# the3cloud/zktls

Hardware: AMD Instinct MI355X
Metric: trace-cells/s (higher is better)
Workload: dtype u32

## Files before the change

### zktls_amd/csrc/context.cpp

```cpp
#include "context.h"
#include "poseidon2.cuh"

#include <atomic>
#include <mutex>
#include <vector>

#include <cstdio>
#include <cstdlib>
#include <cstring>
#include <string>

namespace zk {

extern std::atomic<int> g_live_contexts;

static thread_local std::string g_last_error;

void set_error(const std::string& msg) { g_last_error = msg; }
void fiber_tls_swap_error(std::string& err) { g_last_error.swap(err); }
int fail(int code, const std::string& msg) { g_last_error = msg; return code; }
int hip_fail(hipError_t e, const char* what) {
    g_last_error = std::string("HIP error ") + hipGetErrorName(e) + " (" + hipGetErrorString(e) + ") in " + what;
    (void)hipGetLastError();
    return e == hipErrorOutOfMemory ? ZKHIP_ERR_NOMEM : ZKHIP_ERR_HIP;
// ... 389 lines not shown
        }
        const BigPlan* fp;
        ZK_TRY(get_big_plan(ctx, log_n, 2, st, &fp));
        CombineArgs f = cm[0] ? combine_args(cm[t], width, dst, out_ld, width, log_n, fp) : combine_args(dst, out_ld, dst, out_ld, width, log_n, fp);
        if (cm[0]) { f.in_group_mul = 1; f.in_elem_mul = Np; } else { f.in_group_mul = R; f.in_elem_mul = 1; }
        f.out_group_mul = R; f.out_elem_mul = 1; f.bitrev_out = 1;
        ZK_HIP(launch_ntt_combine(f, ctx->stream));
    }
    return ZKHIP_OK;
}

constexpr int SMALL_LDE_MIN_LOG = 11, SMALL_LDE_MAX_LOG = 15, SMALL_LDE_DEFAULT_MAX_LOG = 13;
constexpr uint32_t SMALL_LDE_MIN_WIDTH = 128;
static int get_small_plan(zkhip_ctx* ctx, int log_n, const SmallPlan** out) {
    for (const SmallPlan& p : ctx->small_plans) if (p.log_n == log_n) { *out = &p; return ZKHIP_OK; }
    SmallPlan p;
    p.log_n = log_n;
    const size_t m = (size_t)1 << (log_n - 5);
    const uint32_t w = two_adic_generator(log_n);
    ZK_HIP(hipMalloc((void**)&p.tw_inv, m * 4));
    if (hipMalloc((void**)&p.tw_fwd, m * 4) != hipSuccess) { (void)hipFree(p.tw_inv); return fail(ZKHIP_ERR_HIP, "hipMalloc (small LDE tables)"); }
    hipError_t e = launch_pow_table(p.tw_inv, m, finv(w), MONTY_R1, ctx->stream);
    if (e == hipSuccess) e = launch_pow_table(p.tw_fwd, m, w, MONTY_R1, ctx->stream);
    if (e != hipSuccess) { (void)hipFree(p.tw_inv); (void)hipFree(p.tw_fwd); return hip_fail(e, "small LDE tables"); }
    ctx->small_plans.push_back(p);
    *out = &ctx->small_plans.back();
    return ZKHIP_OK;
}
static int get_small_pre(zkhip_ctx* ctx, int log_n, uint32_t shift, const uint32_t** out) {
    for (const SmallPre& p : ctx->small_pres) if (p.log_n == log_n && p.shift == shift) { *out = p.pre; return ZKHIP_OK; }
    SmallPre p;
    p.log_n = log_n; p.shift = shift;
    const size_t n = (size_t)1 << log_n;
    ZK_HIP(hipMalloc((void**)&p.pre, n * 4));
    const hipError_t e = launch_pow_table(p.pre, n, shift, finv(to_monty((uint32_t)n)), ctx->stream);
    if (e != hipSuccess) { (void)hipFree(p.pre); return hip_fail(e, "small LDE coset powers"); }
    ctx->small_pres.push_back(p);
    *out = p.pre;
    return ZKHIP_OK;
}
static int lde_small(zkhip_ctx* ctx, const uint32_t* in, size_t in_ld, uint32_t* out, size_t out_ld, int log_n, uint32_t width, int log_blowup,
                     uint32_t shift, bool* done) {
    *done = false;
    if (log_n < SMALL_LDE_MIN_LOG || log_n > SMALL_LDE_MAX_LOG || !ctx->lde_fusion) return ZKHIP_OK;
    int max_log = SMALL_LDE_DEFAULT_MAX_LOG;
    uint32_t min_width = SMALL_LDE_MIN_WIDTH;
#ifdef ZKHIP_AB_HOOKS
    if (const char* e = getenv("ZKHIP_LDE_SMALL")) { max_log = atoi(e); min_width = 1; }
#endif
    if (log_n > max_log || width < min_width) return ZKHIP_OK;
    const size_t n = (size_t)1 << log_n;
    const int B = 1 << log_blowup;
    LdeSmallArgs a{};
    a.in = in; a.in_ld = in_ld; a.out_ld = out_ld; a.ncols = width; a.cosets = (uint32_t)B;
    if (!lde_small_supported(a, log_n)) return ZKHIP_OK;
    const SmallPlan* sp;
    ZK_TRY(get_small_plan(ctx, log_n, &sp));
    a.tw_inv = sp->tw_inv; a.tw_fwd = sp->tw_fwd;
    const uint32_t wnb = two_adic_generator(log_n + log_blowup);
    for (int t = 0; t < B; t++) {
        ZK_TRY(get_small_pre(ctx, log_n, fmul(shift, fpow(wnb, (uint64_t)t)), &a.pre[t]));
        a.out[t] = out + (size_t)reverse_bits((uint32_t)t, log_blowup) * n * out_ld;
    }
    ZK_HIP(launch_lde_small(a, log_n, ctx->stream));
    *done = true;
    return ZKHIP_OK;
}

int op_coset_lde(zkhip_ctx* ctx, const uint32_t* in, size_t in_ld, uint32_t* out, size_t out_ld,
                 int log_n, uint32_t width, int log_blowup, uint32_t shift) {
    if (log_n < 0 || log_n > MAX_LOG_ROWS) return fail(ZKHIP_ERR_INVALID, "coset_lde: log_n must be in [0, 22]");
    if (log_n > BIG_INNER_LOG) {
        if (log_blowup < 0 || log_blowup > 4 || log_n + log_blowup > TWO_ADICITY) return fail(ZKHIP_ERR_INVALID, "coset_lde: bad log_blowup");
        if (width == 0 || in_ld < width || out_ld < width) return fail(ZKHIP_ERR_INVALID, "coset_lde: bad width / ld");
        return coset_lde_big(ctx, in, in_ld, out, out_ld, log_n, width, log_blowup, shift);
    }
    if (log_blowup < 0 || log_blowup > 4 || log_n + log_blowup > TWO_ADICITY) return fail(ZKHIP_ERR_INVALID, "coset_lde: bad log_blowup");
    if (width == 0 || in_ld < width || out_ld < width) return fail(ZKHIP_ERR_INVALID, "coset_lde: bad width / ld");
    if (log_n < 5) {
        void* coef_s;
        ZK_TRY(ctx_reserve(ctx, S_COEF, ((size_t)1 << log_n) * width * 4, &coef_s));
        ZK_HIP(launch_small_eval(in, in_ld, (uint32_t*)coef_s, width, log_n, log_n, width, finv(two_adic_generator(log_n)), MONTY_R1,
                                 finv(to_monty(1u << log_n)), 0, ctx->stream));
        ZK_HIP(launch_small_eval((const uint32_t*)coef_s, width, out, out_ld, log_n, log_n + log_blowup, width,
                                 two_adic_generator(log_n + log_blowup), shift, MONTY_R1, 1, ctx->stream));
        return ZKHIP_OK;
    }
    {
        bool done = false;
        ZK_TRY(lde_small(ctx, in, in_ld, out, out_ld, log_n, width, log_blowup, shift, &done));
        if (done) return ZKHIP_OK;
    }
    if (width > 32 && width % 32 != 0) {
        const uint32_t w32 = width & ~31u;
        ZK_TRY(op_coset_lde(ctx, in, in_ld, out, out_ld, log_n, w32, log_blowup, shift));
        return op_coset_lde(ctx, in + w32, in_ld, out + w32, out_ld, log_n, width - w32, log_blowup, shift);
    }
    const size_t n = (size_t)1 << log_n;
    const int B = 1 << log_blowup;
    int m1, m2;
    split(log_n, &m1, &m2);
    void* coef_v;
    ZK_TRY(ctx_reserve(ctx, S_COEF, n * width * 4, &coef_v));
    uint32_t* coef = (uint32_t*)coef_v;
    const uint32_t wnb = two_adic_generator(log_n + log_blowup);
    if (m1 == 0) {
        ZK_TRY(run_inverse(ctx, in, in_ld, coef, width, log_n, width, false));
        for (int t = 0; t < B; t++) {
            const uint32_t st = fmul(shift, fpow(wnb, (uint64_t)t));
            uint32_t* dst = out + (size_t)reverse_bits((uint32_t)t, log_blowup) * n * out_ld;
            const NttPlan* p;
            ZK_TRY(get_plan(ctx, log_n, 1, st, &p));
            NttPassArgs a = base_args(ctx, coef, width, dst, out_ld, width, false);
            a.num_tiles = 1; a.log_m = log_n; a.in_tile_mul = 0; a.in_stride = 1; a.out_tile_mul = 0; a.out_stride = 1;
            a.pre = p->pre; a.bitrev_out = 1;
            ZK_HIP(launch_ntt_pass(a, false, ctx->stream));
        }
        return ZKHIP_OK;
    }
    uint32_t* dsts[16];
    uint32_t shifts[16];
    for (int t = 0; t < B; t++) {
        shifts[t] = fmul(shift, fpow(wnb, (uint64_t)t));
        dsts[t] = out + (size_t)reverse_bits((uint32_t)t, log_blowup) * n * out_ld;
    }
    return lde_two_pass(ctx, in, in_ld, coef, width, dsts, out_ld, log_n, width, shifts, B);
}

int op_merkle_commit(zkhip_ctx* ctx, const MatDesc* mats, int nmats, int log_h, uint32_t* tree) {
    if (nmats < 1 || nmats > MAX_LEAF_MATS) return fail(ZKHIP_ERR_INVALID, "merkle_commit: 1..8 matrices");
    if (log_h < 0 || log_h > 30) return fail(ZKHIP_ERR_INVALID, "merkle_commit: bad log_h");
    LeafArgs la{};
    for (int m = 0; m < nmats; m++) la.mats[m] = mats[m];
    la.nmats = nmats; la.height = (uint64_t)1 << log_h; la.digests = tree;
    uint32_t* level = tree;
    uint64_t count = la.height;
    if (count > COOP_TOP_NODES && count <= coop_max_nodes()) {
        const uint32_t rest = count >= 4096 ? 128u : 32u;
        ZK_HIP(launch_hash_sub(la, (uint32_t)count / rest, ctx->stream));
        for (uint64_t c = count; c > rest; c >>= 1) level += 8 * c;
        ZK_HIP(launch_compress_top(level, rest, ctx->stream));
        return ZKHIP_OK;
    }
    ZK_HIP(launch_hash_rows(la, ctx->stream));
    while (count > COOP_TOP_NODES) {
        if (count <= coop_max_nodes()) {
            const uint32_t rest = count >= 4096 ? 128u : 32u;
            const uint32_t sub = (uint32_t)count / rest;
            ZK_HIP(launch_compress_sub(level, (uint32_t)count, sub, ctx->stream));
            for (uint64_t c = count; c > rest; c >>= 1) level += 8 * c;
            count = rest;
            break;
        }
        uint32_t* next = level + 8 * count;
        ZK_HIP(launch_compress_level(level, next, count / 2, ctx->stream));
        level = next; count >>= 1;
    }
    ZK_HIP(launch_compress_top(level, (uint32_t)count, ctx->stream));
    return ZKHIP_OK;
}

int op_merkle_commit_mixed(zkhip_ctx* ctx, const MatDesc* mats, const int* log_heights, int nmats, uint32_t* tree) {
    if (nmats < 1 || nmats > 32) return fail(ZKHIP_ERR_INVALID, "merkle_commit_mixed: 1..32 matrices");
    int log_h = 0;
    for (int m = 0; m < nmats; m++) {
        if (log_heights[m] < 0 || log_heights[m] > 30) return fail(ZKHIP_ERR_INVALID, "merkle_commit_mixed: bad height");
        if (log_heights[m] > log_h) log_h = log_heights[m];
    }
    auto gather = [&](int lh, LeafArgs& la) {
        la = LeafArgs{};
        for (int m = 0; m < nmats; m++)
            if (log_heights[m] == lh) {
                if (la.nmats == MAX_LEAF_MATS) return false;
                la.mats[la.nmats++] = mats[m];
            }
        la.height = (uint64_t)1 << lh;
        return true;
    };
    LeafArgs la;
    if (!gather(log_h, la)) return fail(ZKHIP_ERR_INVALID, "merkle_commit_mixed: at most 8 matrices per height");
    if (la.nmats == nmats) return op_merkle_commit(ctx, la.mats, nmats, log_h, tree);
    la.digests = tree;
    ZK_HIP(launch_hash_rows(la, ctx->stream));
    uint32_t* level = tree;
    for (int lvl = log_h - 1; lvl >= 0; lvl--) {
        const uint64_t cnt = (uint64_t)1 << lvl;
        int min_lh = log_h;
        for (int m = 0; m < nmats; m++) if (log_heights[m] < min_lh) min_lh = log_heights[m];
        if (lvl < min_lh && 2 * cnt <= coop_max_nodes()) {
            uint64_t count = 2 * cnt;
            if (count > COOP_TOP_NODES) {
                const uint32_t rest = count >= 4096 ? 128u : 32u;
                ZK_HIP(launch_compress_sub(level, (uint32_t)count, (uint32_t)count / rest, ctx->stream));
                for (uint64_t c = count; c > rest; c >>= 1) level += 8 * c;
                count = rest;
            }
            ZK_HIP(launch_compress_top(level, (uint32_t)count, ctx->stream));
            return ZKHIP_OK;
        }
        uint32_t* next = level + 16 * cnt;
        LeafArgs inj;
        if (!gather(lvl, inj)) return fail(ZKHIP_ERR_INVALID, "merkle_commit_mixed: at most 8 matrices per height");
        if (inj.nmats && compress_inject_ok(inj)) {
            inj.digests = next;
            ZK_HIP(launch_compress_inject(level, inj, ctx->stream));
            level = next;
            continue;
        }
        ZK_HIP(launch_compress_level(level, next, cnt, ctx->stream));
        if (inj.nmats) {
            void* tmp;
            ZK_TRY(ctx_reserve(ctx, S_TMP, cnt * 32, &tmp));
            inj.digests = (uint32_t*)tmp;
            ZK_HIP(launch_hash_rows(inj, ctx->stream));
            ZK_HIP(launch_inject(next, (const uint32_t*)tmp, cnt, ctx->stream));
        }
        level = next;
    }
    return ZKHIP_OK;
}

}

using namespace zk;

extern "C" {

int zkhip_version(void) { return ZKHIP_VERSION; }
const char* zkhip_last_error(void) { return g_last_error.c_str(); }

extern "C++" {
#ifdef ZKHIP_AB_HOOKS
namespace zk {
int logical_devices() {
    static const int k = [] { const char* e = getenv("ZKHIP_LOGICAL_DEVICES"); const int v = e ? atoi(e) : 0; return v > 0 && v <= 64 ? v : 0; }();
    return k;
}
static std::mutex g_alloc_mu;
static std::vector<std::pair<std::pair<uintptr_t, size_t>, int>> g_allocs;
int logical_device_of(const void* p) {
    std::lock_guard<std::mutex> lk(g_alloc_mu);
    const uintptr_t a = (uintptr_t)p;
    for (auto& e : g_allocs) if (a >= e.first.first && a < e.first.first + e.first.second) return e.second;
    return -1;
}
}
#endif
namespace zk {
int physical_device(int device) {
#ifdef ZKHIP_AB_HOOKS
    if (logical_devices() > 0 && device >= 0) {
        int n = 0;
        if (hipGetDeviceCount(&n) != hipSuccess || n <= 0) { (void)hipGetLastError(); return device; }
        return device % n;
    }
#endif
    return device;
}
}
}

int zkhip_device_count(void) {
    int n = 0;
    if (hipGetDeviceCount(&n) != hipSuccess) { (void)hipGetLastError(); return 0; }
#ifdef ZKHIP_AB_HOOKS
    if (n > 0 && logical_devices() > 0) return logical_devices();
#endif
    return n;
}

int zkhip_ctx_create(int device, void* stream, zkhip_ctx** out) {
    if (!out) return fail(ZKHIP_ERR_INVALID, "ctx_create: out is null");
    *out = nullptr;
    int n = 0;
    if (hipGetDeviceCount(&n) != hipSuccess || n <= 0) {
        (void)hipGetLastError();
        return fail(ZKHIP_ERR_NO_DEVICE, "no HIP device visible: libzkhip has no CPU fallback");
    }
    const int logical = device;
#ifdef ZKHIP_AB_HOOKS
    if (logical_devices() > 0) {
        if (device < 0 || device >= logical_devices()) return fail(ZKHIP_ERR_INVALID, "ctx_create: logical device ordinal out of range");
        device = physical_device(device);
    }
#endif
    if (device < 0 || device >= n) return fail(ZKHIP_ERR_INVALID, "ctx_create: device ordinal out of range");
    ZK_HIP(hipSetDevice(device));
    hipDeviceProp_t prop;
    ZK_HIP(hipGetDeviceProperties(&prop, device));
    if (std::strncmp(prop.gcnArchName, "gfx950", 6) != 0)
        return fail(ZKHIP_ERR_NO_DEVICE, std::string("device is ") + prop.gcnArchName + ", libzkhip is built for gfx950 only");
    zkhip_ctx* ctx = new (std::nothrow) zkhip_ctx();
    if (!ctx) return fail(ZKHIP_ERR_NOMEM, "ctx_create: out of host memory");
    g_live_contexts.fetch_add(1);
    ctx->device = device;
    ctx->logical_device = logical;
    if (stream) { ctx->stream = (hipStream_t)stream; ctx->own_stream = false; }
    else {
        hipError_t e = hipStreamCreateWithFlags(&ctx->stream, hipStreamNonBlocking);
        if (e != hipSuccess) { delete ctx; g_live_contexts.fetch_sub(1); return hip_fail(e, "hipStreamCreate"); }
        ctx->own_stream = true;
    }
    int rc = ZKHIP_OK;
    do {
        hipError_t e;
        if ((e = hipMalloc((void**)&ctx->w1024_fwd, 1024 * 4)) != hipSuccess) { rc = hip_fail(e, "hipMalloc"); break; }
        if ((e = hipMalloc((void**)&ctx->w1024_inv, 1024 * 4)) != hipSuccess) { rc = hip_fail(e, "hipMalloc"); break; }
        const uint32_t w = two_adic_generator(10);
        if ((e = launch_pow_table(ctx->w1024_fwd, 1024, w, MONTY_R1, ctx->stream)) != hipSuccess) { rc = hip_fail(e, "pow_table"); break; }
        if ((e = launch_pow_table(ctx->w1024_inv, 1024, finv(w), MONTY_R1, ctx->stream)) != hipSuccess) { rc = hip_fail(e, "pow_table"); break; }
        if ((e = hipMalloc((void**)&ctx->w1024f_fwd, 1024 * 4)) != hipSuccess) { rc = hip_fail(e, "hipMalloc"); break; }
        if ((e = hipMalloc((void**)&ctx->w1024f_inv, 1024 * 4)) != hipSuccess) { rc = hip_fail(e, "hipMalloc"); break; }
        if ((e = launch_fused_table(ctx->w1024f_fwd, ctx->w1024_fwd, 1, 0, ctx->stream)) != hipSuccess) { rc = hip_fail(e, "fused_table"); break; }
        if ((e = launch_fused_table(ctx->w1024f_inv, ctx->w1024_inv, 1, 0, ctx->stream)) != hipSuccess) { rc = hip_fail(e, "fused_table"); break; }
#ifdef ZKHIP_AB_HOOKS
        static P2Tables p2t;
        p2t = g_p2_tables;
        if (getenv("ZKHIP_P2_PER_ROUND")) p2t.pk16.pair = 0;
#else
        const P2Tables& p2t = g_p2_tables;
#endif
        if ((e = hash_upload_p2_tables(p2t, ctx->stream)) != hipSuccess) { rc = hip_fail(e, "upload Poseidon2 tables"); break; }
        if ((e = stark_upload_p2_tables(p2t, ctx->stream)) != hipSuccess) { rc = hip_fail(e, "upload Poseidon2 tables"); break; }
        if ((e = hipStreamSynchronize(ctx->stream)) != hipSuccess) { rc = hip_fail(e, "sync"); break; }
    } while (0);
    if (rc != ZKHIP_OK) { zkhip_ctx_destroy(ctx); return rc; }
    *out = ctx;
    return ZKHIP_OK;
}

void zkhip_ctx_destroy(zkhip_ctx* ctx) {
    if (!ctx) return;
    (void)hipSetDevice(ctx->device);
    if (ctx->stream) (void)hipStreamSynchronize(ctx->stream);
    if (ctx->sha_key) zkhip_machine_key_destroy(ctx->sha_key);
    if (ctx->rec_key) zkhip_machine_key_destroy(ctx->rec_key);
    if (ctx->lift_key) zkhip_machine_key_destroy(ctx->lift_key);
    if (ctx->fri_graph_exec) (void)hipGraphExecDestroy(ctx->fri_graph_exec);
    for (NttPlan& p : ctx->plans) { if (p.pre) (void)hipFree(p.pre); if (p.post) (void)hipFree(p.post); if (p.pre_f) (void)hipFree(p.pre_f); if (p.post_f) (void)hipFree(p.post_f); }
    if (ctx->w1024f_fwd) (void)hipFree(ctx->w1024f_fwd);
    if (ctx->w1024f_inv) (void)hipFree(ctx->w1024f_inv);
    for (BigPlan& p : ctx->big_plans) if (p.tw) (void)hipFree(p.tw);
    for (SmallPlan& p : ctx->small_plans) { if (p.tw_inv) (void)hipFree(p.tw_inv); if (p.tw_fwd) (void)hipFree(p.tw_fwd); }
    for (SmallPre& p : ctx->small_pres) if (p.pre) (void)hipFree(p.pre);
    for (ColPlan& p : ctx->col_plans) { if (p.pre) (void)hipFree(p.pre); if (p.post2d) (void)hipFree(p.post2d); }
    for (DeviceBuffer& b : ctx->scratch) if (b.ptr) (void)hipFree(b.ptr);
    if (ctx->host_pinned) (void)hipHostFree(ctx->host_pinned);
    if (ctx->w1024_fwd) (void)hipFree(ctx->w1024_fwd);
    if (ctx->w1024_inv) (void)hipFree(ctx->w1024_inv);
    for (auto& d : ctx->domains) { (void)hipFree(d.xs); (void)hipFree(d.sel_first); (void)hipFree(d.sel_last); (void)hipFree(d.itw); }
    if (ctx->own_stream && ctx->stream) (void)hipStreamDestroy(ctx->stream);
// ... 342 lines not shown
```

### zktls_amd/csrc/hash.hip

```cpp
#include "poseidon2.cuh"
#include "poseidon2_coop.cuh"
#include "kernels.h"
#include "batch.h"
#include "p24chip.h"
#include "p24chip_rows.cuh"
#include "p2chip.h"

namespace zk {

hipError_t hash_upload_p2_tables(const P2Tables& t, hipStream_t s) { return p2_upload_tables(t, s); }

__device__ __forceinline__ uint32_t load_virtual(const LeafArgs& a, uint64_t row, uint32_t vc) {
    uint32_t off = vc;
#pragma unroll
    for (int m = 0; m < MAX_LEAF_MATS; m++) {
        if (m < a.nmats) {
            if (off < a.mats[m].width) return a.mats[m].ptr[row * a.mats[m].ld + off];
            off -= a.mats[m].width;
        }
    }
    return 0u;
}

__global__ void hash_rows16_kernel(LeafArgs a, uint32_t total_w);
// ... 86 lines not shown
            const uint4 v1 = rp[2 * q + 1];
            s[4] = v1.x; s[5] = v1.y; s[6] = v1.z; s[7] = v1.w;
        }
        p2_permute_mx_form<P2MxForm::SQUEEZE>(s);
    }
    if (row >= height) return;
    uint4* d = reinterpret_cast<uint4*>(digests + row * 8);
    d[0] = make_uint4(s[0], s[1], s[2], s[3]);
    d[1] = make_uint4(s[4], s[5], s[6], s[7]);
}
__device__ __forceinline__ void hash_rows_vec_kernel_body(const uint32_t* __restrict__ mat, uint64_t ld, uint32_t width, uint64_t height, uint32_t* __restrict__ digests) { hash_rows_sponge_body(mat, ld, width, height, digests); }
__global__ void __launch_bounds__(256) __attribute__((amdgpu_waves_per_eu(5))) hash_rows_vec_kernel(const uint32_t* __restrict__ mat, uint64_t ld, uint32_t width, uint64_t height, uint32_t* __restrict__ digests) { hash_rows_vec_kernel_body(mat, ld, width, height, digests); }
struct hash_rows_vec_kernel_bargs { const uint32_t* mat; uint64_t ld; uint32_t width; uint64_t height; uint32_t* digests; static hash_rows_vec_kernel_bargs make(const uint32_t* mat, uint64_t ld, uint32_t width, uint64_t height, uint32_t* digests) { return hash_rows_vec_kernel_bargs{mat, ld, width, height, digests}; } };
__global__ void __launch_bounds__(256) __attribute__((amdgpu_waves_per_eu(5))) hash_rows_vec_kernel_batch(const hash_rows_vec_kernel_bargs* __restrict__ zk_arr) { const hash_rows_vec_kernel_bargs& zk_b = zk_arr[blockIdx.z]; hash_rows_vec_kernel_body(zk_b.mat, zk_b.ld, zk_b.width, zk_b.height, zk_b.digests); }
#ifdef ZKHIP_AB_HOOKS
__global__ void __launch_bounds__(256) hash_rows_vec_valu_kernel(const uint32_t* __restrict__ mat, uint64_t ld, uint32_t width, uint64_t height, uint32_t* __restrict__ digests) { hash_rows_vec_body<false>(mat, ld, width, height, digests); }
__global__ void __launch_bounds__(256) __attribute__((amdgpu_waves_per_eu(5))) hash_rows_vec_closed_kernel(const uint32_t* __restrict__ mat, uint64_t ld, uint32_t width, uint64_t height, uint32_t* __restrict__ digests) { hash_rows_vec_body<true>(mat, ld, width, height, digests); }
#endif

__device__ __forceinline__ void sponge_rows_vec(const LeafArgs& a, uint64_t row, uint32_t total_q, uint32_t s[16]) {
    int m = 0;
    uint32_t q = 0, nq = a.mats[0].width / 4;
    const uint4* rp = reinterpret_cast<const uint4*>(a.mats[0].ptr + row * a.mats[0].ld);
    for (uint32_t b = 0; b < total_q; b += 2) {
        while (q == nq) { m++; q = 0; nq = a.mats[m].width / 4; rp = reinterpret_cast<const uint4*>(a.mats[m].ptr + row * a.mats[m].ld); }
        const uint4 v0 = rp[q++];
        s[0] = v0.x; s[1] = v0.y; s[2] = v0.z; s[3] = v0.w;
        if (b + 1 < total_q) {
            while (q == nq) { m++; q = 0; nq = a.mats[m].width / 4; rp = reinterpret_cast<const uint4*>(a.mats[m].ptr + row * a.mats[m].ld); }
            const uint4 v1 = rp[q++];
            s[4] = v1.x; s[5] = v1.y; s[6] = v1.z; s[7] = v1.w;
        }
        p2_permute_dev(s);
    }
}
__device__ __forceinline__ void hash_rows_mvec_kernel_body(const LeafArgs& a, uint32_t total_q) {
    const uint64_t row = (uint64_t)blockIdx.x * blockDim.x + threadIdx.x;
    if (row >= a.height) return;
    uint32_t s[16];
#pragma unroll
    for (int i = 0; i < 16; i++) s[i] = 0u;
    sponge_rows_vec(a, row, total_q, s);
    uint4* d = reinterpret_cast<uint4*>(a.digests + row * 8);
    d[0] = make_uint4(s[0], s[1], s[2], s[3]);
    d[1] = make_uint4(s[4], s[5], s[6], s[7]);
}
__global__ void __launch_bounds__(256) hash_rows_mvec_kernel(LeafArgs a, uint32_t total_q) { hash_rows_mvec_kernel_body(a, total_q); }
struct hash_rows_mvec_kernel_bargs { LeafArgs a; uint32_t total_q; static hash_rows_mvec_kernel_bargs make(LeafArgs a, uint32_t total_q) { return hash_rows_mvec_kernel_bargs{a, total_q}; } };
__global__ void __launch_bounds__(256) hash_rows_mvec_kernel_batch(const hash_rows_mvec_kernel_bargs* __restrict__ zk_arr) { const hash_rows_mvec_kernel_bargs& zk_b = zk_arr[blockIdx.z]; hash_rows_mvec_kernel_body(zk_b.a, zk_b.total_q); }

__device__ __forceinline__ void compress_inject_mvec_kernel_body(const uint32_t* __restrict__ children, const LeafArgs& a, uint32_t total_q) {
    const uint64_t i = (uint64_t)blockIdx.x * blockDim.x + threadIdx.x;
    if (i >= a.height) return;
    const uint4* cp = reinterpret_cast<const uint4*>(children + 16 * i);
    const uint4 c0 = cp[0], c1 = cp[1], c2 = cp[2], c3 = cp[3];
    uint32_t s[16] = {c0.x, c0.y, c0.z, c0.w, c1.x, c1.y, c1.z, c1.w, c2.x, c2.y, c2.z, c2.w, c3.x, c3.y, c3.z, c3.w};
    uint32_t t[16];
#pragma unroll
    for (int k = 0; k < 16; k++) t[k] = 0u;
    p2_permute_dev(s);
    sponge_rows_vec(a, i, total_q, t);
#pragma unroll
    for (int k = 0; k < 8; k++) s[8 + k] = t[k];
    p2_permute_dev(s);
    uint4* d = reinterpret_cast<uint4*>(a.digests + i * 8);
    d[0] = make_uint4(s[0], s[1], s[2], s[3]);
    d[1] = make_uint4(s[4], s[5], s[6], s[7]);
}
__global__ void __launch_bounds__(256) compress_inject_mvec_kernel(const uint32_t* __restrict__ children, LeafArgs a, uint32_t total_q) { compress_inject_mvec_kernel_body(children, a, total_q); }
struct compress_inject_mvec_kernel_bargs { const uint32_t* children; LeafArgs a; uint32_t total_q; static compress_inject_mvec_kernel_bargs make(const uint32_t* children, LeafArgs a, uint32_t total_q) { return compress_inject_mvec_kernel_bargs{children, a, total_q}; } };
__global__ void __launch_bounds__(256) compress_inject_mvec_kernel_batch(const compress_inject_mvec_kernel_bargs* __restrict__ zk_arr) { const compress_inject_mvec_kernel_bargs& zk_b = zk_arr[blockIdx.z]; compress_inject_mvec_kernel_body(zk_b.children, zk_b.a, zk_b.total_q); }

static bool leaf_mats_vec(const LeafArgs& a) {
    for (int m = 0; m < a.nmats; m++) {
        const MatDesc& d = a.mats[m];
        if (d.width == 0 || d.width % 4 || d.ld % 4 || (reinterpret_cast<uintptr_t>(d.ptr) & 15)) return false;
    }
    return a.nmats >= 1;
}
hipError_t launch_compress_inject(const uint32_t* children, const LeafArgs& a, hipStream_t s) {
    if (a.height == 0) return hipSuccess;
    if (a.nmats < 1 || a.nmats > MAX_LEAF_MATS || !leaf_mats_vec(a)) return hipErrorInvalidValue;
    uint32_t total = 0;
    for (int m = 0; m < a.nmats; m++) total += a.mats[m].width;
    ZK_LAUNCH(compress_inject_mvec_kernel, compress_inject_mvec_kernel_batch, compress_inject_mvec_kernel_bargs, dim3((unsigned)((a.height + 255) / 256)), dim3(256), 0, s, children, a, total / 4);
    return hipGetLastError();
}
bool compress_inject_ok(const LeafArgs& a) { return a.height > coop_max_nodes() && leaf_mats_vec(a); }

hipError_t launch_hash_rows(const LeafArgs& a, hipStream_t s) {
    if (a.height == 0) return hipSuccess;
    if (a.nmats < 1 || a.nmats > MAX_LEAF_MATS) return hipErrorInvalidValue;
    uint32_t total = 0;
    for (int m = 0; m < a.nmats; m++) total += a.mats[m].width;
    if (a.height <= coop_max_nodes()) {
        const uint64_t threads = a.height * 16;
        ZK_LAUNCH(hash_rows16_kernel, hash_rows16_kernel_batch, hash_rows16_kernel_bargs, dim3((unsigned)((threads + 255) / 256)), dim3(256), 0, s, a, total);
        return hipGetLastError();
    }
    dim3 block(256), grid((unsigned)((a.height + 255) / 256));
    const MatDesc& m0 = a.mats[0];
    bool vec = a.nmats == 1 && m0.width % 4 == 0 && m0.ld % 4 == 0 &&
               (reinterpret_cast<uintptr_t>(m0.ptr) & 15) == 0;
#ifdef ZKHIP_AB_HOOKS
    static const bool valu = getenv("ZKHIP_HASH_VEC_VALU") != nullptr;
    if (vec && valu) {
        hash_rows_vec_valu_kernel<<<grid, block, 0, s>>>(m0.ptr, m0.ld, m0.width, a.height, a.digests);
        return hipGetLastError();
    }
    static const bool closed = getenv("ZKHIP_HASH_VEC_CLOSED") != nullptr;
    if (vec && closed) {
        hash_rows_vec_closed_kernel<<<grid, block, 0, s>>>(m0.ptr, m0.ld, m0.width, a.height, a.digests);
        return hipGetLastError();
    }
#endif
    if (vec)
        ZK_LAUNCH(hash_rows_vec_kernel, hash_rows_vec_kernel_batch, hash_rows_vec_kernel_bargs, grid, block, 0, s, m0.ptr, m0.ld, m0.width, a.height, a.digests);
    else if (leaf_mats_vec(a))
        ZK_LAUNCH(hash_rows_mvec_kernel, hash_rows_mvec_kernel_batch, hash_rows_mvec_kernel_bargs, grid, block, 0, s, a, total / 4);
    else
        ZK_LAUNCH(hash_rows_generic_kernel, hash_rows_generic_kernel_batch, hash_rows_generic_kernel_bargs, grid, block, 0, s, a, total);
    return hipGetLastError();
}

__device__ __forceinline__ void compress_node(const uint32_t* children, uint32_t* parent) {
    const uint4* cp = reinterpret_cast<const uint4*>(children);
    uint4 v0 = cp[0], v1 = cp[1], v2 = cp[2], v3 = cp[3];
    uint32_t s[16] = {v0.x, v0.y, v0.z, v0.w, v1.x, v1.y, v1.z, v1.w,
                      v2.x, v2.y, v2.z, v2.w, v3.x, v3.y, v3.z, v3.w};
    p2_permute_dev(s);
    uint4* d = reinterpret_cast<uint4*>(parent);
    d[0] = make_uint4(s[0], s[1], s[2], s[3]);
    d[1] = make_uint4(s[4], s[5], s[6], s[7]);
}

__device__ __forceinline__ void compress_level_kernel_body(const uint32_t* __restrict__ children, uint32_t* __restrict__ parents, uint64_t count) {
    const uint64_t i = (uint64_t)blockIdx.x * blockDim.x + threadIdx.x;
    if (i >= count) return;
    compress_node(children + 16 * i, parents + 8 * i);
}
__global__ void __launch_bounds__(256) compress_level_kernel(const uint32_t* __restrict__ children, uint32_t* __restrict__ parents, uint64_t count) { compress_level_kernel_body(children, parents, count); }
struct compress_level_kernel_bargs { const uint32_t* children; uint32_t* parents; uint64_t count; static compress_level_kernel_bargs make(const uint32_t* children, uint32_t* parents, uint64_t count) { return compress_level_kernel_bargs{children, parents, count}; } };
__global__ void __launch_bounds__(256) compress_level_kernel_batch(const compress_level_kernel_bargs* __restrict__ zk_arr) { const compress_level_kernel_bargs& zk_b = zk_arr[blockIdx.z]; compress_level_kernel_body(zk_b.children, zk_b.parents, zk_b.count); }

hipError_t launch_compress_level(const uint32_t* children, uint32_t* parents, uint64_t count, hipStream_t s) {
    if (count == 0) return hipSuccess;
    if (count <= coop_max_nodes()) {
        const uint64_t threads = count * 16;
        ZK_LAUNCH(compress_level16_kernel, compress_level16_kernel_batch, compress_level16_kernel_bargs, dim3((unsigned)((threads + 255) / 256)), dim3(256), 0, s, children, parents, (uint32_t)count);
        return hipGetLastError();
    }
    ZK_LAUNCH(compress_level_kernel, compress_level_kernel_batch, compress_level_kernel_bargs, dim3((unsigned)((count + 255) / 256)), dim3(256), 0, s, children, parents, count);
    return hipGetLastError();
}

__device__ __forceinline__ void inject_kernel_body(uint32_t* __restrict__ nodes, const uint32_t* __restrict__ extra, uint64_t count) {
    const uint64_t i = (uint64_t)blockIdx.x * blockDim.x + threadIdx.x;
    if (i >= count) return;
    const uint4* a = reinterpret_cast<const uint4*>(nodes + 8 * i);
    const uint4* b = reinterpret_cast<const uint4*>(extra + 8 * i);
    const uint4 v0 = a[0], v1 = a[1], v2 = b[0], v3 = b[1];
    uint32_t s[16] = {v0.x, v0.y, v0.z, v0.w, v1.x, v1.y, v1.z, v1.w, v2.x, v2.y, v2.z, v2.w, v3.x, v3.y, v3.z, v3.w};
    p2_permute_dev(s);
    uint4* d = reinterpret_cast<uint4*>(nodes + 8 * i);
    d[0] = make_uint4(s[0], s[1], s[2], s[3]);
    d[1] = make_uint4(s[4], s[5], s[6], s[7]);
}
__global__ void __launch_bounds__(256) inject_kernel(uint32_t* __restrict__ nodes, const uint32_t* __restrict__ extra, uint64_t count) { inject_kernel_body(nodes, extra, count); }
struct inject_kernel_bargs { uint32_t* nodes; const uint32_t* extra; uint64_t count; static inject_kernel_bargs make(uint32_t* nodes, const uint32_t* extra, uint64_t count) { return inject_kernel_bargs{nodes, extra, count}; } };
__global__ void __launch_bounds__(256) inject_kernel_batch(const inject_kernel_bargs* __restrict__ zk_arr) { const inject_kernel_bargs& zk_b = zk_arr[blockIdx.z]; inject_kernel_body(zk_b.nodes, zk_b.extra, zk_b.count); }

hipError_t launch_inject(uint32_t* nodes, const uint32_t* extra, uint64_t count, hipStream_t s) {
    if (count == 0) return hipSuccess;
    ZK_LAUNCH(inject_kernel, inject_kernel_batch, inject_kernel_bargs, dim3((unsigned)((count + 255) / 256)), dim3(256), 0, s, nodes, extra, count);
    return hipGetLastError();
}

__device__ __forceinline__ void compress_top_kernel_body(uint32_t* tree, uint32_t count) {
    uint32_t* level = tree;
    for (uint32_t n = count; n > 1; n >>= 1) {
        uint32_t* next = level + 8 * (size_t)n;
        for (uint32_t i = threadIdx.x; i < n / 2; i += blockDim.x) compress_node(level + 16 * (size_t)i, next + 8 * (size_t)i);
        __threadfence_block();
        __syncthreads();
        level = next;
    }
}
__global__ void __launch_bounds__(1024) compress_top_kernel(uint32_t* tree, uint32_t count) { compress_top_kernel_body(tree, count); }
struct compress_top_kernel_bargs { uint32_t* tree; uint32_t count; static compress_top_kernel_bargs make(uint32_t* tree, uint32_t count) { return compress_top_kernel_bargs{tree, count}; } };
__global__ void __launch_bounds__(1024) compress_top_kernel_batch(const compress_top_kernel_bargs* __restrict__ zk_arr) { const compress_top_kernel_bargs& zk_b = zk_arr[blockIdx.z]; compress_top_kernel_body(zk_b.tree, zk_b.count); }

hipError_t launch_compress_top(uint32_t* tree, uint32_t count, hipStream_t s) {
    if (count <= 1) return hipSuccess;
    if (count > COOP_TOP_NODES) return hipErrorInvalidValue;
    unsigned threads = count * 8 < 64 ? 64 : (count * 8 > 1024 ? 1024 : count * 8);
    ZK_LAUNCH(compress_top16_kernel, compress_top16_kernel_batch, compress_top16_kernel_bargs, dim3(1), dim3(threads), 0, s, tree, count);
    return hipGetLastError();
}

hipError_t launch_hash_sub(const LeafArgs& a, uint32_t sub, hipStream_t s) {
    if (sub < 2 || (sub & (sub - 1)) || a.height % sub || a.height > COOP_MAX_NODES || a.nmats < 1 || a.nmats > MAX_LEAF_MATS) return hipErrorInvalidValue;
    uint32_t total = 0;
    for (int m = 0; m < a.nmats; m++) total += a.mats[m].width;
    unsigned threads = sub * 8 < 64 ? 64 : (sub * 8 > 1024 ? 1024 : sub * 8);
    ZK_LAUNCH(hash_sub16_kernel, hash_sub16_kernel_batch, hash_sub16_kernel_bargs, dim3((unsigned)(a.height / sub)), dim3(threads), 0, s, a, total, sub);
    return hipGetLastError();
}
hipError_t launch_compress_sub(uint32_t* tree, uint32_t count, uint32_t sub, hipStream_t s) {
    if (sub < 2 || (sub & (sub - 1)) || count % sub || count > COOP_MAX_NODES) return hipErrorInvalidValue;
    unsigned threads = sub * 8 < 64 ? 64 : (sub * 8 > 1024 ? 1024 : sub * 8);
    ZK_LAUNCH(compress_sub16_kernel, compress_sub16_kernel_batch, compress_sub16_kernel_bargs, dim3(count / sub), dim3(threads), 0, s, tree, count, sub);
    return hipGetLastError();
}

__device__ __forceinline__ void compress_level16_kernel_body(const uint32_t* __restrict__ children, uint32_t* __restrict__ parents, uint32_t count) {
    const uint32_t gid = blockIdx.x * blockDim.x + threadIdx.x;
    const uint32_t node = gid >> 4;
    const int lane16 = threadIdx.x & 15;
    if (node >= count) return;
    const CoopConsts k = coop_load_consts(lane16);
    const uint32_t x = coop_permute(children[16 * (size_t)node + lane16], lane16, k);
    if (lane16 < 8) parents[8 * (size_t)node + lane16] = x;
}
__global__ void __launch_bounds__(256) compress_level16_kernel(const uint32_t* __restrict__ children, uint32_t* __restrict__ parents, uint32_t count) { compress_level16_kernel_body(children, parents, count); }
__global__ void __launch_bounds__(256) compress_level16_kernel_batch(const compress_level16_kernel_bargs* __restrict__ zk_arr) { const compress_level16_kernel_bargs& zk_b = zk_arr[blockIdx.z]; compress_level16_kernel_body(zk_b.children, zk_b.parents, zk_b.count); }

__device__ __forceinline__ void compress_top16_kernel_body(uint32_t* tree, uint32_t count) {
    const int lane16 = threadIdx.x & 15;
    const uint32_t grp = threadIdx.x >> 4, ngrp = blockDim.x >> 4;
    const CoopConsts k = coop_load_consts(lane16);
    uint32_t* level = tree;
    for (uint32_t n = count; n > 1; n >>= 1) {
        uint32_t* next = level + 8 * (size_t)n;
        for (uint32_t i = grp; i < n / 2; i += ngrp) {
            const uint32_t x = coop_permute(level[16 * (size_t)i + lane16], lane16, k);
            if (lane16 < 8) next[8 * (size_t)i + lane16] = x;
        }
        __threadfence_block();
        __syncthreads();
        level = next;
    }
}
__global__ void __launch_bounds__(1024) compress_top16_kernel(uint32_t* tree, uint32_t count) { compress_top16_kernel_body(tree, count); }
__global__ void __launch_bounds__(1024) compress_top16_kernel_batch(const compress_top16_kernel_bargs* __restrict__ zk_arr) { const compress_top16_kernel_bargs& zk_b = zk_arr[blockIdx.z]; compress_top16_kernel_body(zk_b.tree, zk_b.count); }

__device__ __forceinline__ void compress_sub16_kernel_body(uint32_t* tree, uint32_t count, uint32_t sub) {
    const int lane16 = threadIdx.x & 15;
    const uint32_t grp = threadIdx.x >> 4, ngrp = blockDim.x >> 4;
    const CoopConsts k = coop_load_consts(lane16);
    uint32_t* level = tree;
    uint32_t n = count, mine = sub;
    while (mine > 1) {
        uint32_t* next = level + 8 * (size_t)n;
        const size_t in0 = (size_t)blockIdx.x * mine, out0 = (size_t)blockIdx.x * (mine / 2);
        for (uint32_t i = grp; i < mine / 2; i += ngrp) {
            const uint32_t x = coop_permute(level[16 * (in0 / 2 + i) + lane16], lane16, k);
            if (lane16 < 8) next[8 * (out0 + i) + lane16] = x;
        }
        __threadfence_block();
        __syncthreads();
        level = next; n >>= 1; mine >>= 1;
    }
}
__global__ void __launch_bounds__(1024) compress_sub16_kernel(uint32_t* tree, uint32_t count, uint32_t sub) { compress_sub16_kernel_body(tree, count, sub); }
__global__ void __launch_bounds__(1024) compress_sub16_kernel_batch(const compress_sub16_kernel_bargs* __restrict__ zk_arr) { const compress_sub16_kernel_bargs& zk_b = zk_arr[blockIdx.z]; compress_sub16_kernel_body(zk_b.tree, zk_b.count, zk_b.sub); }

__device__ __forceinline__ void hash_sub16_kernel_body(const LeafArgs& a, uint32_t total_w, uint32_t sub) {
    const int lane16 = threadIdx.x & 15;
    const uint32_t grp = threadIdx.x >> 4, ngrp = blockDim.x >> 4;
    const CoopConsts k = coop_load_consts(lane16);
    for (uint32_t i = grp; i < sub; i += ngrp) {
        const uint64_t row = (uint64_t)blockIdx.x * sub + i;
        uint32_t x = 0;
        for (uint32_t q = 0; q < total_w; q += 8) {
            if (lane16 < 8 && q + lane16 < total_w) x = load_virtual(a, row, q + lane16);
            x = coop_permute(x, lane16, k);
        }
        if (lane16 < 8) a.digests[row * 8 + lane16] = x;
    }
    __threadfence_block();
    __syncthreads();
    uint32_t* level = a.digests;
    uint32_t n = (uint32_t)a.height, mine = sub;
    while (mine > 1) {
        uint32_t* next = level + 8 * (size_t)n;
        const size_t in0 = (size_t)blockIdx.x * mine, out0 = (size_t)blockIdx.x * (mine / 2);
        for (uint32_t i = grp; i < mine / 2; i += ngrp) {
            const uint32_t x = coop_permute(level[16 * (in0 / 2 + i) + lane16], lane16, k);
            if (lane16 < 8) next[8 * (out0 + i) + lane16] = x;
        }
        __threadfence_block();
        __syncthreads();
        level = next; n >>= 1; mine >>= 1;
    }
}
__global__ void __launch_bounds__(1024) hash_sub16_kernel(LeafArgs a, uint32_t total_w, uint32_t sub) { hash_sub16_kernel_body(a, total_w, sub); }
__global__ void __launch_bounds__(1024) hash_sub16_kernel_batch(const hash_sub16_kernel_bargs* __restrict__ zk_arr) { const hash_sub16_kernel_bargs& zk_b = zk_arr[blockIdx.z]; hash_sub16_kernel_body(zk_b.a, zk_b.total_w, zk_b.sub); }

__device__ __forceinline__ void hash_rows16_kernel_body(const LeafArgs& a, uint32_t total_w) {
    const uint32_t gid = blockIdx.x * blockDim.x + threadIdx.x;
    const uint64_t row = gid >> 4;
    const int lane16 = threadIdx.x & 15;
    if (row >= a.height) return;
    const CoopConsts k = coop_load_consts(lane16);
    uint32_t x = 0;
    for (uint32_t q = 0; q < total_w; q += 8) {
// ... 846 lines not shown
```

### zktls_amd/csrc/kernels.h

```cpp
#pragma once
#include <hip/hip_runtime.h>
#include <stddef.h>
#include <stdint.h>

#include "babybear.cuh"

namespace zk {

struct NttPassArgs {
    const uint32_t* in;
    uint32_t* out;
    uint64_t in_ld, out_ld;
    uint32_t ncols;
    uint32_t num_tiles;
    uint32_t log_m;
    uint64_t in_tile_mul, in_stride;
    uint64_t out_tile_mul, out_stride;
    uint32_t bitrev_out;
    uint32_t map_mode;
    uint64_t tile_perm;
    uint32_t fast_path;
    uint32_t debug_flags;
    uint32_t cols_per_thread;
    uint32_t bench_tag;
    const uint32_t* w1024;
    const uint32_t* pre;
    const uint32_t* post;
};
hipError_t launch_ntt_pass(const NttPassArgs& a, bool inverse, hipStream_t s);

constexpr int FUSED_COSETS = 2;
struct LdeFusedArgs {
    const uint32_t* in;
    uint64_t in_ld, out_ld;
    uint32_t ncols;
    uint32_t num_tiles;
    uint32_t map_rot;
    uint32_t grid;
    uint32_t bench_tag;
    uint64_t in_tile_mul, in_stride;
    uint64_t out_tile_mul, out_stride;
    const uint32_t* w1024_inv;
    const uint32_t* w1024_fwd;
    uint32_t* out[FUSED_COSETS];
    const uint32_t* pre[FUSED_COSETS];
    const uint32_t* post[FUSED_COSETS];
};
hipError_t launch_lde_fused(const LdeFusedArgs& a, hipStream_t s);
hipError_t launch_fused_table(uint32_t* out, const uint32_t* in, uint32_t blocks, int mode, hipStream_t s);
bool lde_fused_supported(const LdeFusedArgs& a);

struct LdeSmallArgs {
    const uint32_t* in;
    uint64_t in_ld, out_ld;
    uint32_t ncols;
    uint32_t cosets;
    uint32_t groups;
    uint32_t reserved;
    const uint32_t* tw_inv;
    const uint32_t* tw_fwd;
    uint32_t* out[16];
    const uint32_t* pre[16];
};
bool lde_small_supported(const LdeSmallArgs& a, int log_n);
hipError_t launch_lde_small(const LdeSmallArgs& a, int log_n, hipStream_t s);

struct ColPassArgs {
    const uint32_t* in;
    uint32_t* out;
    uint64_t in_batch, out_batch;
    uint32_t count;
    uint32_t tload, tstore, in_brev, out_brev;
    const uint32_t* w1024;
    const uint32_t* pre;
    const uint32_t* post2d;
};
hipError_t launch_ntt_colpass(const ColPassArgs& a, bool inverse, hipStream_t s);
hipError_t launch_post2d_table(uint32_t* out, uint32_t w, uint32_t shift, uint32_t scale, hipStream_t s);

struct CombineArgs {
    const uint32_t* in;
    uint32_t* out;
    uint64_t in_ld, out_ld;
    uint32_t ncols;
    uint64_t groups;
    int log_r;
    uint64_t in_group_mul, in_elem_mul, out_group_mul, out_elem_mul;
    int bitrev_out;
    int inverse;
    const uint32_t* tw;
};
hipError_t launch_ntt_combine(const CombineArgs& a, hipStream_t s);
hipError_t launch_combine_table(uint32_t* out, uint32_t rows, uint64_t groups, uint32_t w, uint32_t shift, uint32_t scale, int bits, hipStream_t s);

hipError_t launch_pow_table(uint32_t* out, size_t n, uint32_t base, uint32_t scale, hipStream_t s);
hipError_t launch_post_table(uint32_t* out, uint32_t rows, uint32_t cols, uint32_t omega,
                             uint32_t shift, uint32_t scale, hipStream_t s);

struct MatDesc {
    const uint32_t* ptr;
    uint64_t ld;
    uint32_t width;
};
constexpr int MAX_LEAF_MATS = 8;
constexpr uint32_t COOP_MAX_NODES = 16384;
uint32_t coop_max_nodes();
constexpr uint32_t COOP_TOP_NODES = 512;
struct LeafArgs {
    MatDesc mats[MAX_LEAF_MATS];
    int nmats;
    uint64_t height;
    uint32_t* digests;
};
hipError_t launch_hash_rows(const LeafArgs& a, hipStream_t s);
hipError_t launch_compress_level(const uint32_t* children, uint32_t* parents, uint64_t count,
                                 hipStream_t s);
hipError_t launch_inject(uint32_t* nodes, const uint32_t* extra, uint64_t count, hipStream_t s);
bool compress_inject_ok(const LeafArgs& a);
hipError_t launch_compress_inject(const uint32_t* children, const LeafArgs& a, hipStream_t s);
hipError_t launch_compress_top(uint32_t* tree, uint32_t count, hipStream_t s);
hipError_t launch_compress_sub(uint32_t* tree, uint32_t count, uint32_t sub, hipStream_t s);
hipError_t launch_hash_sub(const LeafArgs& a, uint32_t sub, hipStream_t s);
hipError_t launch_merkle_p24_colmajor(const uint32_t* mat, uint32_t cols, int log_rows, uint32_t* tree, hipStream_t s);
hipError_t launch_merkle_p24_rowmajor(const uint32_t* mat, uint64_t ld, uint32_t width, int log_rows, uint32_t* tree, hipStream_t s);
struct P2Tables;
hipError_t hash_upload_p2_tables(const P2Tables& t, hipStream_t s);
hipError_t stark_upload_p2_tables(const P2Tables& t, hipStream_t s);
namespace p2chip { struct MerkleTraceArgs; struct LayerPathsArgs; struct P2RArgs; struct MrecChainArgs; struct Fri16TranscriptArgs; }
hipError_t launch_p2chip_merkle(const p2chip::MerkleTraceArgs& a, hipStream_t s);
namespace p24chip { struct MerkleTraceArgs; struct LayerPathsArgs; struct RowPathsArgs; }
hipError_t launch_p24chip_merkle(const p24chip::MerkleTraceArgs& a, hipStream_t s);
hipError_t launch_p24chip_row_paths(const p24chip::RowPathsArgs& a, hipStream_t s);
hipError_t launch_p24chip_layer_paths(const p24chip::LayerPathsArgs& a, hipStream_t s);
hipError_t launch_fri16_transcript(const p2chip::Fri16TranscriptArgs& a, hipStream_t s);
hipError_t launch_p2chip_layer_paths(const p2chip::LayerPathsArgs& a, hipStream_t s);
hipError_t launch_mrec_chains(const p2chip::MrecChainArgs& a, hipStream_t s);
hipError_t launch_p2r_rows(const p2chip::P2RArgs& a, hipStream_t s);
hipError_t launch_permute_states(uint32_t* states, uint64_t count, hipStream_t s);

hipError_t launch_fill_uniform(uint32_t* out, uint64_t ld, uint64_t seed, uint64_t rows,
                               uint32_t width, hipStream_t s);
hipError_t launch_gen_trace(uint32_t* out, uint64_t ld, uint64_t seed, uint64_t rows,
                            uint32_t width, hipStream_t s);
hipError_t launch_gen_trace_logup(uint32_t* out, uint64_t ld, uint64_t seed, uint64_t rows, uint32_t width, uint32_t pairs,
                                  uint64_t recv_seed, uint32_t recv_width, hipStream_t s);
hipError_t launch_small_eval(const uint32_t* in, uint64_t in_ld, uint32_t* out, uint64_t out_ld, int log_n, int log_out, uint32_t width,
                             uint32_t w, uint32_t shift, uint32_t scale, int bitrev_out, hipStream_t s);
hipError_t launch_transpose(const uint32_t* in, uint32_t* out, uint64_t rows, uint64_t cols, int rev_bits_in, int rev_bits_out, hipStream_t s);
hipError_t launch_convert(const uint32_t* in, uint32_t* out, uint64_t n, bool to_monty_form,
                          hipStream_t s);

hipError_t launch_domain_tables(uint32_t* xs, uint32_t* sel_first, uint32_t* sel_last, uint32_t* itw, int log_n, int log_blowup, hipStream_t s);

struct QuotientArgs {
    const uint32_t* lde;
    uint64_t ld;
    uint32_t width;
    int log_n;
    int lanes_per_row;
    const uint32_t* xs;
    const uint32_t* sel_first;
    uint32_t wn_inv;
    uint32_t inv_zh_even, inv_zh_odd;
    const uint32_t* alpha_pow;
    uint32_t pairs;
    const uint32_t* perm;
    uint64_t perm_ld;
    Ext gamma, beta;
    Ext cumsum;
    const uint32_t* sel_last;
    uint32_t* addend_out;
    const uint32_t* addend;
    uint32_t* out;
    uint32_t* lde_out;
    uint64_t lde_ld;
};
hipError_t launch_quotient(const QuotientArgs& a, hipStream_t s);
hipError_t launch_logup_addend(const QuotientArgs& a, hipStream_t s);

constexpr uint32_t AIR_SLOT_EXTRA = 4;
constexpr uint32_t AIR_GP = 36;
#if defined(__HIPCC__)
__host__ __device__
#endif
inline uint32_t air_lds_base(uint32_t slot, uint32_t W) {
    if (slot < W) return AIR_GP * (slot >> 2) + (slot & 3u);
    if (slot < 2 * W) { const uint32_t c = slot - W; return AIR_GP * (c >> 2) + (c & 3u) + 4u; }
    const uint32_t x = slot - 2 * W;
    return AIR_GP * ((W >> 2) + (x >> 2)) + (x & 3u);
}
struct QuotientAirArgs {
    const uint32_t* lde; uint64_t ld; uint32_t width; int log_n;
    const uint32_t* xs; const uint32_t* sel_first; const uint32_t* sel_last;
    uint32_t wn_inv;
    int log_qd;
    uint32_t inv_zh[4];
    const uint32_t* body;
    uint32_t n_constraints;
    const uint32_t* weights;
    const uint32_t* pub;
    uint32_t* out;
    uint32_t* lde_out; uint64_t lde_ld;
    const uint32_t* recs; uint32_t n_terms; uint32_t n_public;
    const uint32_t* addend;
    uint32_t no_chain;
    uint32_t wide;
    uint32_t cls[6];
};
constexpr uint32_t AIR_WIDE_POINTS = 64, AIR_WIDE_PITCH = 65;
inline bool air_wide_form(uint32_t width, uint32_t n_terms, int log_n, uint32_t n_public) {
    return n_terms >= 2048 && width % 4 == 0 && (size_t)AIR_WIDE_PITCH * (width + AIR_SLOT_EXTRA + n_public) * 4 <= 160 * 1024 && log_n >= 6;
}
ZK_HD uint32_t air_wide_word(uint32_t slot, uint32_t W) {
    if (slot < W) return AIR_WIDE_PITCH * slot;
    if (slot < 2 * W) return AIR_WIDE_PITCH * (slot - W) + 1u;
    return AIR_WIDE_PITCH * (W + (slot - 2 * W));
}
hipError_t launch_quotient_air(const QuotientAirArgs& a, hipStream_t s);

hipError_t launch_inv_denominators(const uint32_t* xs, uint64_t count, const Ext& z0, const Ext& z1, int npoints,
                                   uint32_t* out, uint32_t* xw, uint64_t xw_count, hipStream_t s);

struct OpenArgs {
    const uint32_t* mat;
    uint64_t ld;
    uint32_t width;
    uint64_t rows;
    const uint32_t* xw;
    uint64_t xw_stride;
    uint32_t* partial;
    int tx;
};
size_t open_chunks(uint64_t rows, uint32_t width, uint64_t ld, const uint32_t* mat);
hipError_t launch_open(const OpenArgs& a, int npts, const Ext& scale0, const Ext& scale1, uint32_t* out, hipStream_t s);

struct ReducedArgs {
    const uint32_t* tlde; uint64_t t_ld; uint32_t width;
    const uint32_t* qlde; uint64_t q_ld; uint32_t q_width;
    const uint32_t* plde; uint64_t p_ld; uint32_t p_width;
    uint64_t rows;
    const uint32_t* alpha_pow;
    const uint32_t* dinv;
    Ext y_loc, y_next, y_pl, y_pn, y_q, off_next, off_pl, off_pn, off_q;
    Ext off_loc;
    int accumulate;
    uint32_t* out;
};
hipError_t launch_reduced_opening(const ReducedArgs& a, uint32_t* scratch_at, hipStream_t s);
int rowdot_form(uint32_t width, uint64_t rows);

struct PermArgs {
    const uint32_t* trace; uint64_t ld;
    uint64_t rows; uint32_t pairs;
    Ext gamma, beta;
    uint32_t* out; uint64_t out_ld;
};
hipError_t launch_perm_trace(const PermArgs& a, uint32_t* block_scratch, hipStream_t s);

constexpr int LOOKUP_REC_WORDS = 12;
struct LookupArgs {
    const uint32_t* table; uint32_t ni, cols;
    Ext gamma, bpow[9];
    const uint8_t* cmap; uint32_t n_used, chunk_mask;
};
constexpr uint32_t LOOKUP_MAX_COLS = 512, LOOKUP_STAGE_MAX_USED = 56;
struct MachinePermArgs {
    LookupArgs lk;
    const uint32_t* trace; uint64_t ld; uint64_t rows;
    uint32_t* out; uint64_t out_ld;
// ... 48 lines not shown
```

Baseline: 21.33 billion.

## Fuse up to three Merkle compress levels per launch using LDS

Adds a kernel that compresses one to three Merkle tree levels in a single launch. Each workgroup hashes 256 pairs, passes the parents through shared memory, and hashes the next levels with fewer active threads. The plain commit path and the mixed-height path, for runs of levels without injected matrices, now use it instead of one launch per level. This cuts kernel launches and avoids re-reading parent digests from global memory, at the cost of idle lanes in the upper levels and extra barriers.

```diff
diff --git a/zktls_amd/csrc/context.cpp b/zktls_amd/csrc/context.cpp
--- a/zktls_amd/csrc/context.cpp
+++ b/zktls_amd/csrc/context.cpp
@@ -565,9 +565,9 @@
             count = rest;
             break;
         }
-        uint32_t* next = level + 8 * count;
-        ZK_HIP(launch_compress_level(level, next, count / 2, ctx->stream));
-        level = next; count >>= 1;
+        const int lv = compress_levels_step(count, 30);
+        ZK_HIP(launch_compress_levels(level, count, lv, ctx->stream));
+        for (int l = 0; l < lv; l++) { level += 8 * count; count >>= 1; }
     }
     ZK_HIP(launch_compress_top(level, (uint32_t)count, ctx->stream));
     return ZKHIP_OK;
@@ -589,6 +589,10 @@
             }
         la.height = (uint64_t)1 << lh;
         return true;
+    };
+    auto injected = [&](int lh) {
+        for (int m = 0; m < nmats; m++) if (log_heights[m] == lh) return true;
+        return false;
     };
     LeafArgs la;
     if (!gather(log_h, la)) return fail(ZKHIP_ERR_INVALID, "merkle_commit_mixed: at most 8 matrices per height");
@@ -610,6 +614,14 @@
             }
             ZK_HIP(launch_compress_top(level, (uint32_t)count, ctx->stream));
             return ZKHIP_OK;
+        }
+        int plain = 0;
+        while (plain <= lvl && !injected(lvl - plain)) plain++;
+        if (const int lv = compress_levels_step(2 * cnt, plain)) {
+            ZK_HIP(launch_compress_levels(level, 2 * cnt, lv, ctx->stream));
+            for (int l = 0; l < lv; l++) level += (size_t)16 << (lvl - l);
+            lvl -= lv - 1;
+            continue;
         }
         uint32_t* next = level + 16 * cnt;
         LeafArgs inj;
diff --git a/zktls_amd/csrc/hash.hip b/zktls_amd/csrc/hash.hip
--- a/zktls_amd/csrc/hash.hip
+++ b/zktls_amd/csrc/hash.hip
@@ -262,6 +262,132 @@
     }
     ZK_LAUNCH(compress_level_kernel, compress_level_kernel_batch, compress_level_kernel_bargs, dim3((unsigned)((count + 255) / 256)), dim3(256), 0, s, children, parents, count);
     return hipGetLastError();
+}
+
+template <bool MX>
+__device__ __forceinline__ void compress_state(uint32_t s[16], uint32_t* parent) {
+    if (MX) p2_permute_mx_dev(s); else p2_permute_dev(s);
+    uint4* d = reinterpret_cast<uint4*>(parent);
+    d[0] = make_uint4(s[0], s[1], s[2], s[3]);
+    d[1] = make_uint4(s[4], s[5], s[6], s[7]);
+}
+__device__ __forceinline__ void load_pair(const uint4* cp, uint32_t s[16]) {
+    const uint4 v0 = cp[0], v1 = cp[1], v2 = cp[2], v3 = cp[3];
+    s[0] = v0.x; s[1] = v0.y; s[2] = v0.z; s[3] = v0.w; s[4] = v1.x; s[5] = v1.y; s[6] = v1.z; s[7] = v1.w;
+    s[8] = v2.x; s[9] = v2.y; s[10] = v2.z; s[11] = v2.w; s[12] = v3.x; s[13] = v3.y; s[14] = v3.z; s[15] = v3.w;
+}
+__device__ __forceinline__ void join_left(uint32_t s[16], const uint32_t left[8]) {
+#pragma unroll
+    for (int k = 0; k < 8; k++) { s[8 + k] = s[k]; s[k] = left[k]; }
+}
+template <int LV, bool MX>
+__device__ __forceinline__ void compress_levels3_regs(uint32_t* level, uint64_t count) {
+    const uint64_t i = (uint64_t)blockIdx.x * blockDim.x + threadIdx.x;
+    if (i >= (count >> LV)) return;
+    uint32_t* const l1 = level + 8 * count;
+    uint32_t* const l2 = l1 + 4 * count;
+    uint32_t* const l3 = l2 + 2 * count;
+    const uint4* cp = reinterpret_cast<const uint4*>(level + 8 * (i << LV));
+    uint32_t s[16], p0[8], g0[8];
+#pragma unroll 1
+    for (int a = 0; a < (LV == 3 ? 2 : 1); a++) {
+#pragma unroll 1
+        for (int b = 0; b < (LV >= 2 ? 2 : 1); b++) {
+            const int k = 2 * a + b;
+            load_pair(cp + 4 * k, s);
+            compress_state<MX>(s, l1 + 8 * ((i << (LV - 1)) + k));
+            if (LV >= 2 && b == 0) {
+#pragma unroll
+                for (int q = 0; q < 8; q++) p0[q] = s[q];
+            }
+        }
+        if (LV >= 2) {
+            join_left(s, p0);
+            compress_state<MX>(s, l2 + 8 * ((i << (LV - 2)) + a));
+            if (LV == 3 && a == 0) {
+#pragma unroll
+                for (int q = 0; q < 8; q++) g0[q] = s[q];
+            }
+        }
+    }
+    if (LV == 3) {
+        join_left(s, g0);
+        compress_state<MX>(s, l3 + 8 * i);
+    }
+}
+template <int LV, bool MX>
+__device__ __forceinline__ void compress_levels3_lds(uint32_t* level, uint64_t count) {
+    __shared__ uint4 sh1[LV >= 2 ? 512 : 1], sh2[LV == 3 ? 256 : 1];
+    const uint32_t t = threadIdx.x;
+    const uint64_t wg = blockIdx.x;
+    if (wg * 512 >= count) return;
+    uint32_t* const l1 = level + 8 * count;
+    uint32_t* const l2 = l1 + 4 * count;
+    uint32_t* const l3 = l2 + 2 * count;
+    uint32_t s[16];
+    load_pair(reinterpret_cast<const uint4*>(level + 16 * (wg * 256 + t)), s);
+    compress_state<MX>(s, l1 + 8 * (wg * 256 + t));
+    if (LV == 1) return;
+    sh1[2 * t] = make_uint4(s[0], s[1], s[2], s[3]);
+    sh1[2 * t + 1] = make_uint4(s[4], s[5], s[6], s[7]);
+    __syncthreads();
+    if (t >= 128) return;
+    load_pair(sh1 + 4 * t, s);
+    compress_state<MX>(s, l2 + 8 * (wg * 128 + t));
+    if (LV == 2) return;
+    sh2[2 * t] = make_uint4(s[0], s[1], s[2], s[3]);
+    sh2[2 * t + 1] = make_uint4(s[4], s[5], s[6], s[7]);
+    __syncthreads();
+    if (t >= 64) return;
+    load_pair(sh2 + 4 * t, s);
+    compress_state<MX>(s, l3 + 8 * (wg * 64 + t));
+}
+constexpr int LEVELS3_FORM = 3;
+template <int LV, int FORM>
+__device__ __forceinline__ void compress_levels3_kernel_body(uint32_t* level, uint64_t count) {
+    if (FORM & 2) compress_levels3_lds<LV, (FORM & 1) != 0>(level, count); else compress_levels3_regs<LV, (FORM & 1) != 0>(level, count);
+}
+template <int LV, int FORM>
+__global__ void __launch_bounds__(256) __attribute__((amdgpu_waves_per_eu(5))) compress_levels3_kernel(uint32_t* level, uint64_t count) { compress_levels3_kernel_body<LV, FORM>(level, count); }
+struct compress_levels3_kernel_bargs { uint32_t* level; uint64_t count; static compress_levels3_kernel_bargs make(uint32_t* level, uint64_t count) { return compress_levels3_kernel_bargs{level, count}; } };
+template <int LV, int FORM>
+__global__ void __launch_bounds__(256) __attribute__((amdgpu_waves_per_eu(5))) compress_levels3_kernel_batch(const compress_levels3_kernel_bargs* __restrict__ zk_arr) { const compress_levels3_kernel_bargs& zk_b = zk_arr[blockIdx.z]; compress_levels3_kernel_body<LV, FORM>(zk_b.level, zk_b.count); }
+
+template <int FORM>
+static hipError_t launch_compress_levels_form(uint32_t* level, uint64_t count, int levels, hipStream_t s) {
+    const dim3 grid((unsigned)(FORM & 2 ? count / 512 : ((count >> levels) + 255) / 256)), block(256);
+    if (levels == 1) ZK_LAUNCH((compress_levels3_kernel<1, FORM>), (compress_levels3_kernel_batch<1, FORM>), compress_levels3_kernel_bargs, grid, block, 0, s, level, count);
+    else if (levels == 2) ZK_LAUNCH((compress_levels3_kernel<2, FORM>), (compress_levels3_kernel_batch<2, FORM>), compress_levels3_kernel_bargs, grid, block, 0, s, level, count);
+    else ZK_LAUNCH((compress_levels3_kernel<3, FORM>), (compress_levels3_kernel_batch<3, FORM>), compress_levels3_kernel_bargs, grid, block, 0, s, level, count);
+    return hipGetLastError();
+}
+hipError_t launch_compress_levels(uint32_t* level, uint64_t count, int levels, hipStream_t s) {
+    if (levels < 1 || levels > 3 || (count & (count - 1)) || (count >> levels) < 256 || count > ((uint64_t)1 << 31)) return hipErrorInvalidValue;
+#ifdef ZKHIP_AB_HOOKS
+    static const int form = getenv("ZKHIP_LEVELS3_FORM") ? atoi(getenv("ZKHIP_LEVELS3_FORM")) : LEVELS3_FORM;
+    if (form < 0) {
+        for (int l = 0; l < levels; l++, level += 8 * count, count >>= 1) {
+            const hipError_t e = launch_compress_level(level, level + 8 * count, count / 2, s);
+            if (e != hipSuccess) return e;
+        }
+        return hipSuccess;
+    }
+    if (form != LEVELS3_FORM) {
+        switch (form) {
+            case 0: return launch_compress_levels_form<0>(level, count, levels, s);
+            case 1: return launch_compress_levels_form<1>(level, count, levels, s);
+            case 2: return launch_compress_levels_form<2>(level, count, levels, s);
+            case 3: return launch_compress_levels_form<3>(level, count, levels, s);
+            default: return hipErrorInvalidValue;
+        }
+    }
+#endif
+    return launch_compress_levels_form<LEVELS3_FORM>(level, count, levels, s);
+}
+int compress_levels_step(uint64_t count, int max_levels) {
+    int total = 0;
+    while (total < max_levels && (count >> total) > coop_max_nodes()) total++;
+    return total % 3 ? total % 3 : (total ? 3 : 0);
 }
 
 __device__ __forceinline__ void inject_kernel_body(uint32_t* __restrict__ nodes, const uint32_t* __restrict__ extra, uint64_t count) {
diff --git a/zktls_amd/csrc/kernels.h b/zktls_amd/csrc/kernels.h
--- a/zktls_amd/csrc/kernels.h
+++ b/zktls_amd/csrc/kernels.h
@@ -115,6 +115,8 @@
 hipError_t launch_hash_rows(const LeafArgs& a, hipStream_t s);
 hipError_t launch_compress_level(const uint32_t* children, uint32_t* parents, uint64_t count,
                                  hipStream_t s);
+hipError_t launch_compress_levels(uint32_t* level, uint64_t count, int levels, hipStream_t s);
+int compress_levels_step(uint64_t count, int max_levels);
 hipError_t launch_inject(uint32_t* nodes, const uint32_t* extra, uint64_t count, hipStream_t s);
 bool compress_inject_ok(const LeafArgs& a);
 hipError_t launch_compress_inject(const uint32_t* children, const LeafArgs& a, hipStream_t s);
```

After: 21.19 billion. No clear change (-0.7%).
